# skitzoid/Box2D-MT

Measured on AMD Instinct MI355X. Metric: world steps/sec at 99858 bodies per GPU (BASELINE config 3: Tumbler 100k, CCD off; Step = collide + island solve + broad-phase + state read-back); for N > 1: container-steps/s = world steps/s x N containers in the one sharded world, higher is better.
Workload: dtype f32

## Files before the change

### box2d-mt_amd/csrc/b2d_kernels_broadphase.h

```cpp
#ifndef B2D_KERNELS_BROADPHASE_H
#define B2D_KERNELS_BROADPHASE_H

#include "b2d_kernels_solve_large.h"

#define SYNC_TILE 1024
__global__ __launch_bounds__(256) void k_sync_fixtures(DW W)
{
	b2dPhaseStamp(W);
	DState* S = W.st;
	const int n = W.nProxies;
	const int tid = (int)threadIdx.x;
	__shared__ int s_list[SYNC_TILE];
	__shared__ int s_cnt, s_base;
	const int perLane = n >= 262144 ? SYNC_TILE / 256 : 1, tile = 256 * perLane;
	if (blockIdx.x == 0 && tid == 0) S->c.gridFresh = 0;
	for (int base = blockIdx.x * tile; base < n; base += gridDim.x * tile)
	{
		if (tid == 0) s_cnt = 0;
		__syncthreads();
		for (int j = 0; j < perLane; ++j)
		{
			const int p = base + j * 256 + tid;
			if (p >= n) break;
			const int body = W.p_body[p];
// ... 124 lines not shown
			int ix, iy;
			proxyCell(W, a, &ix, &iy);
			atomicAdd(&W.gridCount[cellHash(ix, iy, W.gridMask)], 1);
		}
	}
}

__global__ __launch_bounds__(256) void k_grid_fill(DW W, int force)
{
	b2dPhaseStamp(W);
	DState* S = W.st;
	if (S->c.nMoves == 0 && !force) return;
	if (force == 1 && S->c.gridFresh) return;
	const int n = W.nProxies;
	for (int p = blockIdx.x * blockDim.x + threadIdx.x; p < n; p += gridDim.x * blockDim.x)
	{
		if (W.p_body[p] < 0) continue;
		float4 a = W.p_fat[p];
		if (proxyIsLarge(W, a)) continue;
		int ix, iy;
		proxyCell(W, a, &ix, &iy);
		uint32_t h = cellHash(ix, iy, W.gridMask);
		const int slot = W.gridStart[h] + atomicAdd(&W.gridCursor[h], 1);
		W.gridItems[slot] = p;
		W.gridFat[slot] = a;
	}
}

__device__ __forceinline__ bool pairPasses(const DW& W, int p, int q, uint64_t* keyOut, int2* proxOut)
{
	const int bodyP = W.p_body[p], bodyQ = W.p_body[q];
	if (bodyP == bodyQ) return false;
	if (W.spatial)
	{
		const bool mineP = (W.b_flags[bodyP] & BF_TYPE_MASK) != BT_STATIC && W.b_owner[bodyP] == (uint8_t)W.shardRank;
		const bool mineQ = (W.b_flags[bodyQ] & BF_TYPE_MASK) != BT_STATIC && W.b_owner[bodyQ] == (uint8_t)W.shardRank;
		if (!mineP && !mineQ) return false;
	}
	const int keyP = W.p_key[p], keyQ = W.p_key[q];
	const int lo = keyP < keyQ ? p : q;
	const int hi = keyP < keyQ ? q : p;
	const uint64_t key = ((uint64_t)(uint32_t)W.p_key[lo] << 32) | (uint32_t)W.p_key[hi];
	if (htContains(W, key + 1ull)) return false;
	if (!bodiesShouldCollide(W, W.p_body[hi], W.p_body[lo])) return false;
	if (!W.userFilter && !filterShouldCollide(W.p_filter0[lo], W.p_filter1[lo], W.p_filter0[hi], W.p_filter1[hi])) return false;
	if (b2dContactSwap(W.shapes[W.p_shape[lo]].type, W.shapes[W.p_shape[hi]].type) < 0) return false;
	*keyOut = key;
	*proxOut = make_int2(lo, hi);
	return true;
}

__device__ __forceinline__ void tryEmitPair(const DW& W, DState* S, int p, int q)
{
	uint64_t key;
	int2 prox;
	if (!pairPasses(W, p, q, &key, &prox)) return;
	int k = atomicAdd(&S->c.nPairs, 1);
	if (k < W.capPairs)
	{
		W.pairKey[k] = key;
		W.pairProxy[k] = prox;
	}
	else
	{
		atomicOr(&S->c.overflow, 2);
	}
}

#define PAIR_STAGE_CAP 256
struct PairStage
{
	uint64_t* key;
	int2* prox;
	int n;
// ... 39 lines not shown
	__syncthreads();
	pairStageStore(W, S, st, lane, s_stageBase + s_stageCount[wv]);
	st.n = 0;
}

struct PairHits
{
	int2* list;
	int n;
};
__device__ __forceinline__ void pairHitsFlush(const DW& W, DState* S, PairHits& h, PairStage& st, int lane)
{
	if (h.n == 0) return;
	if (st.n + h.n > PAIR_STAGE_CAP) pairStageDrain(W, S, st, lane);
	__builtin_amdgcn_fence(__ATOMIC_RELEASE, "wavefront");
	__builtin_amdgcn_wave_barrier();
	__builtin_amdgcn_fence(__ATOMIC_ACQUIRE, "wavefront");
	uint64_t key = 0ull;
	int2 prox = make_int2(0, 0);
	bool ok = false;
	if (lane < h.n)
	{
		const int2 pq = h.list[lane];
		ok = pairPasses(W, pq.x, pq.y, &key, &prox);
	}
	const unsigned long long om = __ballot(ok);
	if (ok)
	{
		const int j = st.n + (int)__popcll(om & ((1ull << lane) - 1ull));
		st.key[j] = key;
		st.prox[j] = prox;
	}
	st.n += (int)__popcll(om);
	__builtin_amdgcn_wave_barrier();
	h.n = 0;
}
__device__ __forceinline__ void pairHitsAdd(const DW& W, DState* S, PairHits& h, PairStage& st, int lane, bool hit, int p, int q)
{
	const unsigned long long hm = __ballot(hit);
	if (hm == 0ull) return;
	const int more = (int)__popcll(hm);
	if (h.n + more > 64) pairHitsFlush(W, S, h, st, lane);
	if (hit) h.list[h.n + (int)__popcll(hm & ((1ull << lane) - 1ull))] = make_int2(p, q);
	h.n += more;
}

__global__ __launch_bounds__(256) void k_find_pairs_small(DW W)
{
	b2dPhaseStamp(W);
	DState* S = W.st;
	const int nm = S->c.nMoves < W.capMoves ? S->c.nMoves : W.capMoves;
	const int nLarge = S->c.nLargeProxies;
	const int lane = (int)(threadIdx.x & 63u);
	const int waveId = (int)((blockIdx.x * blockDim.x + threadIdx.x) >> 6);
	const int nWaves = (int)((gridDim.x * blockDim.x) >> 6);
	int rounds = 0;
	__shared__ int2 s_hits[4][64];
	__shared__ uint64_t s_stageKey[4][PAIR_STAGE_CAP];
	__shared__ int2 s_stageProx[4][PAIR_STAGE_CAP];
	PairHits hits;
	hits.list = s_hits[threadIdx.x >> 6];
	hits.n = 0;
	PairStage stage;
	stage.key = s_stageKey[threadIdx.x >> 6];
	stage.prox = s_stageProx[threadIdx.x >> 6];
	stage.n = 0;
	const int largeQ = lane < nLarge ? W.largeProxies[lane] : -1;
	const float4 largeFat = largeQ >= 0 ? W.p_fat[largeQ] : make_float4(0, 0, 0, 0);
	auto cellHeaders = [&](const float4& f, int* cntOut, int* startOut)
	{
// ... 49 lines not shown
		for (int c = 0; c < 9; ++c)
		{
			ccs[c] = __builtin_amdgcn_readlane(cnt, c);
			scs[c] = __builtin_amdgcn_readlane(start, c);
			ecs[c] = total;
			total += ccs[c];
		}
		{ const int r = (total + 63) >> 6; rounds += r < 8 ? r : 8; }
		for (int base = 0; base < total; base += 64)
		{
			const int idx = base + lane;
			const bool valid = idx < total;
			int t = -1;
#pragma unroll
			for (int c = 0; c < 9; ++c)
			{
				const int ec = ecs[c], cc = ccs[c], sc = scs[c];
				if (valid && idx >= ec && idx < ec + cc) t = sc + (idx - ec);
			}
			bool hit = false;
			int q = -1;
			if (t >= 0)
			{
				q = W.gridItems[t];
				const float4 fq = W.gridFat[t];
				AABB bq;
				bq.lo = v2(fq.x, fq.y);
				bq.hi = v2(fq.z, fq.w);
				hit = q != p && b2dAabbOverlap(a, bq);
			}
			pairHitsAdd(W, S, hits, stage, lane, hit, p, q);
		}
		{
			AABB bq;
			bq.lo = v2(largeFat.x, largeFat.y);
			bq.hi = v2(largeFat.z, largeFat.w);
			pairHitsAdd(W, S, hits, stage, lane, largeQ >= 0 && b2dAabbOverlap(a, bq), p, largeQ);
		}
		for (int t = 64 + lane; t < nLarge; t += 64)
		{
			const int q = W.largeProxies[t];
			if (b2dAabbOverlap(a, loadAabb(W.p_fat, q))) tryEmitPair(W, S, p, q);
		}
	}
	pairHitsFlush(W, S, hits, stage, lane);
	pairStageFinish(W, S, stage, lane);
	b2dBlockTreeAdd2(W, ARRIVE_PAIRS, &S->c.candRounds[0], lane == 0 ? rounds : 0, &S->c.candRounds[1], 0, (unsigned)W.capMoves <= (TREE_SUM_MAX >> 3));
}


__global__ __launch_bounds__(256) void k_find_pairs_window(DW W)
{
	b2dPhaseStamp(W);
	DState* S = W.st;
	const int nm = S->c.nMoves < W.capMoves ? S->c.nMoves : W.capMoves;
	const int nLarge = S->c.nLargeProxies;
	const int lane = (int)(threadIdx.x & 63u);
	const int waveId = (int)((blockIdx.x * blockDim.x + threadIdx.x) >> 6);
	const int nWaves = (int)((gridDim.x * blockDim.x) >> 6);
	int rounds = 0;
	__shared__ int2 s_hits[4][64];
	__shared__ uint64_t s_stageKey[4][PAIR_STAGE_CAP];
	__shared__ int2 s_stageProx[4][PAIR_STAGE_CAP];
	PairHits hits;
	hits.list = s_hits[threadIdx.x >> 6];
	hits.n = 0;
	PairStage stage;
	stage.key = s_stageKey[threadIdx.x >> 6];
	stage.prox = s_stageProx[threadIdx.x >> 6];
	stage.n = 0;
	const int largeQ = lane < nLarge ? W.largeProxies[lane] : -1;
	const float4 largeFat = largeQ >= 0 ? W.p_fat[largeQ] : make_float4(0, 0, 0, 0);
	int pNext = waveId < nm ? W.moveBuf[waveId] : -1;
	int pAhead = waveId + nWaves < nm ? W.moveBuf[waveId + nWaves] : -1;
// ... 41 lines not shown
		{ const int r = (total + 63) >> 6; rounds += r < 8 ? r : 8; }
		for (int base = 0; base < total; base += 64)
		{
			const int idx = base + lane;
			const bool valid = idx < total;
			int t = -1;
			{
				int lo = 0, hi = nCells - 1;
#pragma unroll
				for (int step = 0; step < 6; ++step)
				{
					const int mid = (lo + hi) >> 1;
					const int im = __shfl(incl, mid);
					if (im > idx) hi = mid; else lo = mid + 1;
				}
				const int c = lo < 63 ? lo : 63;
				const int ec = __shfl(excl, c), sc = __shfl(start, c);
				if (valid) t = sc + (idx - ec);
			}
			bool hit = false;
			int q = -1;
			if (t >= 0)
			{
				q = W.gridItems[t];
				const float4 fq = W.gridFat[t];
				AABB bq;
				bq.lo = v2(fq.x, fq.y);
				bq.hi = v2(fq.z, fq.w);
				hit = q != p && b2dAabbOverlap(a, bq);
			}
			pairHitsAdd(W, S, hits, stage, lane, hit, p, q);
		}
		{
			AABB bq;
			bq.lo = v2(largeFat.x, largeFat.y);
			bq.hi = v2(largeFat.z, largeFat.w);
			pairHitsAdd(W, S, hits, stage, lane, largeQ >= 0 && b2dAabbOverlap(a, bq), p, largeQ);
		}
		for (int t = 64 + lane; t < nLarge; t += 64)
		{
			const int q = W.largeProxies[t];
			if (b2dAabbOverlap(a, loadAabb(W.p_fat, q))) tryEmitPair(W, S, p, q);
		}
	}
	pairHitsFlush(W, S, hits, stage, lane);
	pairStageFinish(W, S, stage, lane);
	b2dBlockTreeAdd2(W, ARRIVE_PAIRS, &S->c.candRounds[0], lane == 0 ? rounds : 0, &S->c.candRounds[1], 0, (unsigned)W.capMoves <= (TREE_SUM_MAX >> 3));
}

__global__ __launch_bounds__(256) void k_find_pairs_large(DW W)
{
	b2dPhaseStamp(W);
// ... 456 lines not shown
```

### box2d-mt_amd/csrc/b2d_kernels_query.h

```cpp
#ifndef B2D_KERNELS_QUERY_H
#define B2D_KERNELS_QUERY_H

#include "b2d_kernels_broadphase.h"
#include "b2d_kernels_collide.h"
#include "b2d_shapecast.h"
#include "b2d_shape_geom.h"

#define QUERY_WINDOW_MAX 4096
#define QUERY_COORD_MAX 1.0e8f
#define QUERY_SORT_MAX 4096
#define QUERY_SORT_THREADS 256

__device__ __forceinline__ bool queryFilterPasses(const DW& W, int q, uint32_t mask, int sensors)
{
	return (W.p_filter0[q] & mask & 0xffffu) != 0u && (sensors || (W.p_filter1[q] & PF_SENSOR) == 0);
}

__device__ __forceinline__ bool queryBoxSane(float4 b)
{
	return fabsf(b.x) <= QUERY_COORD_MAX && fabsf(b.y) <= QUERY_COORD_MAX && fabsf(b.z) <= QUERY_COORD_MAX && fabsf(b.w) <= QUERY_COORD_MAX;
}

__device__ __forceinline__ unsigned long long queryKey(uint32_t valueBits, int q)
{
// ... 57 lines not shown
			const int v = __shfl_up(incl, off);
			if (lane >= off) incl += v;
		}
		const int excl = incl - cnt;
		const int total = __shfl(incl, 63);
		for (int base = 0; base < total; base += 64)
		{
			const int idx = base + lane;
			int lo = 0, hi = 63;
#pragma unroll
			for (int step = 0; step < 6; ++step)
			{
				const int mid = (lo + hi) >> 1;
				if (__shfl(incl, mid) > idx) hi = mid; else lo = mid + 1;
			}
			const int cl = lo < 63 ? lo : 63;
			const int t = __shfl(start, cl) + (idx - __shfl(excl, cl));
			const int cellX = __shfl(cx, cl), cellY = __shfl(cy, cl);
			bool valid = idx < total;
			int q = -1;
			float4 fat = make_float4(0.0f, 0.0f, 0.0f, 0.0f);
			if (valid)
			{
				q = W.gridItems[t];
				fat = W.gridFat[t];
				int px, py;
				proxyCell(W, fat, &px, &py);
				valid = px == cellX && py == cellY;
			}
			visit(valid, q, fat);
		}
	}
	return true;
}

template <typename F>
__device__ __forceinline__ void queryVisitLarge(const DW& W, int lane, F& visit)
{
	const int nLarge = W.st->c.nLargeProxies;
	for (int base = 0; base < nLarge; base += 64)
	{
		const int k = base + lane;
		const int q = k < nLarge ? W.largeProxies[k] : -1;
		visit(q >= 0, q, q >= 0 ? W.p_fat[q] : make_float4(0.0f, 0.0f, 0.0f, 0.0f));
	}
}

// ... 666 lines not shown
```

### box2d-mt_amd/csrc/b2d_kernels_toi.h

```cpp
#ifndef B2D_KERNELS_TOI_H
#define B2D_KERNELS_TOI_H

#include "b2d_kernels_broadphase.h"
#include "b2d_toi.h"

#define TOI_LANES 512
#define TOI_CAND_MAX 512
#define TOI_MOVES_MAX 128
#define TOI_PAIRS_MAX 512
#define TOI_RECOMP_MAX 512
#define TOI_WOKEN_MAX 256
#define TOI_EVENTS_MAX 100000
#define TOI_NEWPAIR_MAX 256
#define TOI_MOVED_ALL_MAX 32768

__device__ __forceinline__ uint32_t ldFlags(const uint32_t* p)
{
	return __hip_atomic_load(p, __ATOMIC_RELAXED, __HIP_MEMORY_SCOPE_AGENT);
}

__device__ __forceinline__ Sweep loadSweep(const DW& W, int body)
{
	const float4 p0 = W.b_pos0[body], p = W.b_pos[body], m = W.b_mass[body];
	Sweep s;
	s.localCenter = v2(m.z, m.w);
	s.c0 = v2(p0.x, p0.y);
	s.a0 = p0.z;
	s.alpha0 = p0.w;
	s.c = v2(p.x, p.y);
	s.a = p.z;
	return s;
}

template <typename F>
__device__ __forceinline__ void toiForEachCandidate(const DW& W, AABB a, int lane, int nLanes, const int* moved, int nMoved, F f)
{
	int ix0, iy0, nx, ny;
	if (!gridWindow(W, make_float4(a.lo.x, a.lo.y, a.hi.x, a.hi.y), &ix0, &iy0, &nx, &ny))
	{
		for (int q = lane; q < W.nProxies; q += nLanes) f(q);
		return;
	}
	const int nCells = nx * ny;
	for (int c = lane; c < nCells; c += nLanes)
	{
		const uint32_t h = cellHash(ix0 + c % nx, iy0 + c / nx, W.gridMask);
		const int start = W.gridStart[h], n = W.gridCount[h];
		for (int t = 0; t < n; ++t) f(W.gridItems[start + t]);
	}
	const int nLarge = W.st->c.nLargeProxies;
	for (int t = lane; t < nLarge; t += nLanes) f(W.largeProxies[t]);
	for (int t = lane; t < nMoved; t += nLanes) f(moved[t]);
}

__device__ __forceinline__ float computeToiOf(const GjkProxy& pA, const GjkProxy& pB, const Sweep& sA, const Sweep& sB)
{
	float t = 1.0f;
	const int state = b2dTimeOfImpact(&t, pA, sA, pB, sB, 1.0f);
	const float alpha0 = sA.alpha0;
	return state == TOI_TOUCHING ? b2dMin(alpha0 + (1.0f - alpha0) * t, 1.0f) : 1.0f;
}
__device__ __forceinline__ float computeToi(const DW& W, int4 ids, const Sweep& sA, const Sweep& sB)
{
	const GjkProxy pA = b2dProxy(W.shapes + W.p_shape[ids.x]);
	const GjkProxy pB = b2dProxy(W.shapes + W.p_shape[ids.y]);
	float t = 1.0f;
	const int state = b2dTimeOfImpact(&t, pA, sA, pB, sB, 1.0f);
	const float alpha0 = sA.alpha0;
	return state == TOI_TOUCHING ? b2dMin(alpha0 + (1.0f - alpha0) * t, 1.0f) : 1.0f;
}

// ... 1211 lines not shown
```

### box2d-mt_amd/csrc/b2d_kernels_toi_chains.h

```cpp
#ifndef B2D_KERNELS_TOI_CHAINS_H
#define B2D_KERNELS_TOI_CHAINS_H

#include "b2d_kernels_toi.h"

#define CHAIN_LANES 64
#define CHAIN_CAND_MAX 64
#define CHAIN_EVENTS_MAX 4096
#define CHAIN_ADJ_MAX 32
#define TOI_GROUPS_MAX 262144

#define TOI_UNSAFE_PARTNER 1
#define TOI_UNSAFE_WOKE 2
#define TOI_UNSAFE_PAIR 4
#define TOI_UNSAFE_CAPACITY 8
#define TOI_UNSAFE_MOVED 16

__global__ __launch_bounds__(256) void k_toi_groups_begin(DW W)
{
	b2dPhaseStamp(W);
	DState* S = W.st;
	const int n = S->c.nToiList < W.capContacts ? S->c.nToiList : W.capContacts;
	const ContactArrays& C = W.ca[S->cur];
	for (int k = blockIdx.x * blockDim.x + threadIdx.x; k < n; k += gridDim.x * blockDim.x)
	{
// ... 778 lines not shown
			if (events) atomicAdd(&S->c.nToiEvents, (int)events);
			if (calls) atomicAdd(&S->c.nToiCalls, (int)calls);
		}
		toiChainsEnd(W);
	}
}

__global__ __launch_bounds__(256) void k_bp_clear(DW W)
{
	b2dPhaseStamp(W);
	DState* S = W.st;
	if (blockIdx.x == 0 && threadIdx.x == 0)
	{
		S->c.nLargeProxies = 0;
		S->c.nLargeMoves = 0;
		S->c.nPairs = 0;
		S->c.nNewContacts = 0;
		S->c.nMovesSeen = S->c.nMoves;
		S->c.gridFresh = S->c.nMoves != 0 ? 1 : 0;
	}
	if (blockIdx.x == 0 && threadIdx.x < 32) S->c.candRounds[threadIdx.x] = 0;
	if (S->c.nMoves == 0) return;
	const uint32_t stride = gridDim.x * blockDim.x, t0 = blockIdx.x * blockDim.x + threadIdx.x;
	{
		const float cap = 4.0f * W.cellSize;
		float ext = 0.0f;
		for (uint32_t p = t0; p < (uint32_t)W.nProxies; p += stride)
		{
			if (W.p_body[p] < 0) continue;
			const float4 a = W.p_fat[p];
			const float e = fmaxf(a.z - a.x, a.w - a.y);
			if (e <= cap && e > ext) ext = e;
		}
		blockAtomicMaxIfAbove((int*)&S->c.cellExtBits, ext > 0.0f ? (int)__float_as_uint(ext) : 0);
	}
	{
		const int4 z = make_int4(0, 0, 0, 0);
		int4* gc = (int4*)W.gridCount;
		int4* gu = (int4*)W.gridCursor;
		for (uint32_t i = t0, n4 = (W.gridMask + 1u) >> 2; i < n4; i += stride)
		{
			gc[i] = z;
			gu[i] = z;
		}
		if (keysetDecision(W) != 0)
		{
// ... 42 lines not shown
```

### box2d-mt_amd/csrc/b2d_world.h

```cpp
#ifndef B2D_WORLD_H
#define B2D_WORLD_H

#include "b2d_solver.h"
#include "b2d_joint.h"
#include "b2d_wave.h"

#define BF_TYPE_MASK 0x3u
#define BF_AWAKE 0x4u
#define BF_AUTOSLEEP 0x8u
#define BF_BULLET 0x10u
#define BF_FIXEDROT 0x20u
#define BF_ACTIVE 0x40u
#define BF_ISLAND 0x80u
#define BF_LARGE 0x100u

#define BT_STATIC 0u
#define BT_KINEMATIC 1u
#define BT_DYNAMIC 2u

#define CF_TOUCHING 0x1u
#define CF_ENABLED 0x2u
#define CF_FILTER 0x4u
#define CF_TOI_CANDIDATE 0x8u
#define CF_SENSOR 0x10u
// ... 369 lines not shown
	int4* spTailKey;
	int userFilter;
	int preSolveOn, postSolveOn;
	float4* pre_o0;
	float4* pre_o1;
	float4* pre_oimp;
	int4* pre_o3;
	PreSolveRec* preRecs;
	PostSolveRec* postRecs;
	ToiLogRec* toiLog;
	int capToiLog;
	int toiEventCap;
	int toiContinue;
	const int4* toiVerdict;
	int nToiVerdict;
	int* filterList;

	int* moveBuf;
	int* gridCount;
	int* gridStart;
	int* gridCursor;
	unsigned long long* arriveTree;
	int* gridItems;
	float4* gridFat;
	int* largeProxies;
	int* largeMoves;
	uint64_t* pairKey;
	int2* pairProxy;
	uint64_t* pairKey2;
	int2* pairProxy2;
	int* pairFirst;
	int* pairRank;

	int* toiList;
	int* toiPos2c;
	int* toiDestroyList;
	int* toiNewList;
	int* b_toiGroup;
	int* toiGroups;
	int* toiParent;
	int* toiDomOf;
	int* toiDomRoot;
	int* toiDomCount;
	int* toiDomBase;
	int* toiDomFill;
	int* toiDomList;
	int* toiDomFailed;
	int* toiDomEvents;
	float4* toiHull;
	int* toiGroupCount;
	int* toiGroupList;
	int* toiMoved;
	int gridHalf;
	int noOwnIdBlocks;
	int noChainCreate;
	int* toiNew;
	float4* snapBody;
	float4* snapFat;

	int* scanTmp;
	int* radixHist;
	int* keepFlag;
	int* keepScan;

	float* stateOut;
};

#if defined(__HIPCC__)
__host__ __device__ inline bool b2dPartitionSettled(const Counters& c)
{
	if (c.nBlocks == 0 || c.nOrphanRows > 0 || c.blkMaxRows > c.blkLanes || c.blkMaxBodies > c.blkLanes || c.nSerialOrphans > 2048) return false;
	if (c.partitionAge > 240 && (4 * c.nCutRows > c.nLContacts || 2 * c.nLContacts < 900)) return false;
	return true;
}

__device__ __forceinline__ void b2dStoreAgentI(int* p, int v) { __hip_atomic_store(p, v, __ATOMIC_RELAXED, __HIP_MEMORY_SCOPE_AGENT); }
__device__ __forceinline__ int b2dLoadAgentI(const int* p) { return __hip_atomic_load(p, __ATOMIC_RELAXED, __HIP_MEMORY_SCOPE_AGENT); }
__device__ __forceinline__ void b2dStoreAgent4(float4* p, float4 v)
{
	typedef float f4 __attribute__((ext_vector_type(4)));
	f4 q;
	q.x = v.x; q.y = v.y; q.z = v.z; q.w = v.w;
	asm volatile("global_store_dwordx4 %0, %1, off sc1\n\ts_nop 1" :: "v"(p), "v"(q) : "memory");
}
__device__ __forceinline__ float4 b2dLoadAgent4(const float4* p)
{
	typedef float f4 __attribute__((ext_vector_type(4)));
	f4 r;
	asm volatile("global_load_dwordx4 %0, %1, off sc1\n\ts_waitcnt vmcnt(0)" : "=v"(r) : "v"(p) : "memory");
	return make_float4(r.x, r.y, r.z, r.w);
}
// ... 119 lines not shown
```

### box2d-mt_amd/csrc/b2hip_api_callbacks.h

```cpp

int b2hip_set_contact_filter(b2hip_world* w, b2hip_should_collide_fn fn, void* user)
{
	if (int rcu = checkUsable(w, "b2hip_set_contact_filter", true)) return rcu;
	w->filterFn = fn;
	w->filterUser = user;
	w->dw.userFilter = hasFilter(w) ? 1 : 0;
	return B2HIP_OK;
}

int b2hip_set_contact_filter_batch(b2hip_world* w, b2hip_should_collide_batch_fn fn, void* user)
{
	if (int rcu = checkUsable(w, "b2hip_set_contact_filter_batch", true)) return rcu;
	w->filterBatchFn = fn;
	if (fn) w->filterUser = user;
	w->dw.userFilter = hasFilter(w) ? 1 : 0;
	return B2HIP_OK;
}

int b2hip_default_should_collide(b2hip_world* w, int fixture_a, int fixture_b)
{
	if (!w || fixture_a < 0 || fixture_b < 0 || fixture_a >= (int)w->fixtures.size() || fixture_b >= (int)w->fixtures.size())
		return setError(B2HIP_ERR_INVALID, "bad fixture id");
	const HostFixture& a = w->fixtures[fixture_a];
	const HostFixture& b = w->fixtures[fixture_b];
// ... 212 lines not shown
	case 31:
	{
		if (first != 0 || count != 1) return setError(B2HIP_ERR_INVALID, "island-build statistics: [0, 1)");
		memcpy(out, &w->statUnionSkipped, sizeof(long long));
		return 0;
	}
	case 29:
	{
		if (first != 0 || count != 1) return setError(B2HIP_ERR_INVALID, "lifecycle statistics: [0, 1)");
		memcpy(out, &w->statLifecycleLongSorts, sizeof(long long));
		return 0;
	}
	case 30:
	{
		const long long stats[2] = { w->statFixtureLongSorts, w->statFixtureRelists };
		if (first < 0 || count < 0 || first + count > 2) return setError(B2HIP_ERR_INVALID, "fixture-batch statistics: [0, 2)");
		memcpy(out, stats + first, (size_t)count * sizeof(long long));
		return 0;
	}
	case 32:
	{
		if (first != 0 || count != 1) return setError(B2HIP_ERR_INVALID, "body-property statistics: [0, 1)");
		memcpy(out, &w->statBodyPropRefits, sizeof(long long));
		return 0;
	}
	case 25:
	{
		if (first < 0 || count < 0 || first + count > ToiStats::N) return setError(B2HIP_ERR_INVALID, "TOI host statistics: [0, 10)");
		memcpy(out, w->toiStats.n + first, (size_t)count * sizeof(long long));
		return 0;
	}
	case 26:
	{
		const int nb = (int)std::min(w->bodies.size(), w->upBodies);
		if (first < 0 || count < 0 || first + count > nb) return setError(B2HIP_ERR_INVALID, "effective blocks: [0, uploaded bodies)");
		if (count == 0) return 0;
		if (!w->d_state.p || !w->b_blk1.p || !w->b_adopt.p || !w->b_flags.p) return setError(B2HIP_ERR_INVALID, "effective blocks: nothing uploaded yet");
		Counters c;
		HIP_TRY(hipMemcpy(&c, &w->d_state.p->c, sizeof(Counters), hipMemcpyDeviceToHost));
		std::vector<int> blk1((size_t)count), adopt((size_t)count);
		std::vector<uint32_t> flags((size_t)count);
		HIP_TRY(hipMemcpy(blk1.data(), w->b_blk1.p + first, (size_t)count * sizeof(int), hipMemcpyDeviceToHost));
		HIP_TRY(hipMemcpy(adopt.data(), w->b_adopt.p + first, (size_t)count * sizeof(int), hipMemcpyDeviceToHost));
		HIP_TRY(hipMemcpy(flags.data(), w->b_flags.p + first, (size_t)count * sizeof(uint32_t), hipMemcpyDeviceToHost));
		const int blocks = c.nBlocks < MAX_BLOCKS ? c.nBlocks : MAX_BLOCKS;
		const bool ownIdOff = (w->dw.nJoints != 0 || c.maxDegree > HUB_DEGREE) && w->dw.noOwnIdBlocks >= 0;
// ... 309 lines not shown
```

### box2d-mt_amd/csrc/b2hip_api_snapshot.h

```cpp

namespace
{
struct SnapHeader
{
	char magic[8];
	uint32_t version, szDState, szHostBody, szHostFixture, szShape, szJoint;
	uint32_t nBodies, nFixtures, nShapes, nJoints, nFree, nContacts, nToiOrder, nMoves;
	uint32_t stateCount, cur;
	int32_t nextNode, leafCount, lastContacts, newFixture;
	float inv_dt0, cellSize;
	int32_t eventsOn, solverHints;
};
const uint32_t kSnapVersion = 6;
const char kSnapMagic[8] = { 'B', '2', 'H', 'I', 'P', 'S', 'N', '1' };

struct SnapWriter
{
	std::vector<char> out;
	void host(const void* p, size_t n) { const char* c = (const char*)p; out.insert(out.end(), c, c + n); }
	int dev(const void* p, size_t n)
	{
		const size_t at = out.size();
		out.resize(at + n);
		if (n == 0) return 0;
// ... 260 lines not shown
	w->gears.resize(nG);
	if (nG) memcpy((void*)w->gears.data(), gearsAt, nG * sizeof(GearRec));
	w->nextNode = h.nextNode; w->leafCount = h.leafCount; w->lastContacts = h.lastContacts; w->newFixture = h.newFixture != 0;
	w->inv_dt0 = h.inv_dt0;
	w->eventsOn = h.eventsOn != 0;
	w->serialOrphansNext = h.solverHints & 1;
	w->blocksTooBig = (h.solverHints & 2) != 0;
	w->stepComplete = (h.solverHints & 4) == 0;
	w->adoptSticky = (h.solverHints >> 8) & 0xff;
	w->largeHintSteps = (h.solverHints >> 16) & 0xff;
	w->recolorCountdown = (h.solverHints >> 24) & 0x7f;
	w->freshColors = ((h.solverHints >> 3) & 0x1f) | ((int)(((uint32_t)h.solverHints >> 31) & 1u) << 5);
	w->freshColorsPending = false;
	w->adoptPasses = w->adoptSticky > 0;
	rc = ensureCapacity(w, nC);
	if (rc) return fail(rc);
	if (nM > w->moveBuf.cap || nC > (size_t)w->dw.capContacts || (size_t)h.stateCount * 10 > w->h_stateCap) return fail(corrupt("counts exceed the buffers sized for them"));
	if (h.stateCount) memcpy(w->h_state, stateAt, (size_t)h.stateCount * 10 * sizeof(float));
	w->shadowDev = nullptr;
	w->stateCount = h.stateCount;
	*w->h_dstate = ds;
	w->contactsKnown = false;
	forestDrop(w);
#define SNAP_UP(arr, s) do { if ((s).bytes && hipMemcpy(w->arr.p, (s).p, (s).bytes, hipMemcpyHostToDevice) != hipSuccess) return fail(setError(B2HIP_ERR_HIP, "snapshot upload failed (" #arr ")")); } while (0)
	if (hipMemcpy(w->d_state.p, &ds, sizeof(DState), hipMemcpyHostToDevice) != hipSuccess) return fail(setError(B2HIP_ERR_HIP, "snapshot upload failed (state block)"));
	w->pubSeq = ds.pubCount;
	SNAP_UP(b_pos, sPos); SNAP_UP(b_pos0, sPos0); SNAP_UP(b_vel, sVel); SNAP_UP(b_xf, sXf); SNAP_UP(b_mass, sMass); SNAP_UP(b_damp, sDamp);
	w->forceOnDevice = true; w->rowsWentEarly = false;
	SNAP_UP(b_force, sForce); SNAP_UP(b_flags, sFlags); SNAP_UP(b_wake, sWake); SNAP_UP(b_proxyHead, sHead); SNAP_UP(b_blk1, sBlk);
	SNAP_UP(p_fat, sFat); SNAP_UP(p_body, sPBody); SNAP_UP(p_shape, sPShape); SNAP_UP(p_key, sPKey); SNAP_UP(p_filter0, sF0); SNAP_UP(p_filter1, sF1);
	SNAP_UP(p_mat, sPMat); SNAP_UP(p_next, sNext);
	const int cur = (int)h.cur;
	SNAP_UP(c_ids[cur], cIds); SNAP_UP(c_key[cur], cKey); SNAP_UP(c_flags[cur], cFlags); SNAP_UP(c_mat[cur], cMat); SNAP_UP(c_man0[cur], cMan0);
	SNAP_UP(c_man1[cur], cMan1); SNAP_UP(c_imp[cur], cImp); SNAP_UP(c_man3[cur], cMan3); SNAP_UP(c_color[cur], cColor); SNAP_UP(c_mgr[cur], cMgr);
	SNAP_UP(toiPos2c, sToi); SNAP_UP(moveBuf, sMoves);
#undef SNAP_UP
	if (nS && hipMemcpy(w->d_shapes.p, w->shapes.data(), nS * sizeof(ShapeRec), hipMemcpyHostToDevice) != hipSuccess)
		return fail(setError(B2HIP_ERR_HIP, "snapshot upload failed (shapes)"));
	w->upBodies = nb; w->upFixtures = np; w->upShapes = nS; w->upJoints = 0;
	w->dw.cellSize = h.cellSize;
	w->dw.invCellSize = 1.0f / h.cellSize;
	w->dw.eventsOn = w->eventsOn ? 1 : 0;
	*out = w;
	return B2HIP_OK;
}

// ... 48 lines not shown
```

### box2d-mt_amd/csrc/b2hip_host_phases.h

```cpp

static int spExchangeState(b2hip_world* w, int mode);
static int spExchangePairs(b2hip_world* w, long long* totalPairs, int* straddling);
static int spResolve(b2hip_world* w, int nVirt = 0);
static int spAfterToi(b2hip_world* w);
static int spBeginStep(b2hip_world* w);

static int radixBits(int maxKey)
{
	int bits = 1;
	while ((1 << bits) <= maxKey && bits < 31) ++bits;
	return bits;
}

static void radixPasses(int first, int bits, std::vector<std::pair<int, int>>& out)
{
	const int passes = (bits + RADIX_BITS - 1) / RADIX_BITS;
	for (int p = 0, at = 0; p < passes; ++p)
	{
		const int width = (bits - at + (passes - p) - 1) / (passes - p);
		out.push_back(std::make_pair(first + at, width));
		at += width;
	}
}

// ... 140 lines not shown
	if (c.overflow & 2) w->pairCapHint = 2 * (size_t)c.nPairs + 4096;
	int rc = ensureCapacity(w, (size_t)c.nContacts + (size_t)std::max(c.nNewContacts, 0) + 1024);
	if (rc) return rc;
	HIP_TRY(hipMemsetAsync(&w->d_state.p->c.overflow, 0, sizeof(int), w->stream));
	return 0;
}

static int findNewContacts(b2hip_world* w, bool sync)
{
	w->contactsKnown = false;
	forestDrop(w);
	for (int attempt = 0; sync && attempt < 4; ++attempt)
	{
		int rc = findNewContactsOnce(w, true);
		if (rc != 1) return rc;
	}
	if (sync) return setError(B2HIP_ERR_CAPACITY, "pair buffer overflow");
	return findNewContactsOnce(w, false);
}

static int findNewContactsOnce(b2hip_world* w, bool sync)
{
	DW& d = w->dw;
	LAUNCH(w, k_bp_clear, gridFor(std::max(d.htMask, d.gridMask) + 1), 256, d);
	LAUNCH(w, k_bp_build, gridFor(std::max(d.capContacts, d.nProxies)), 256, d);
	deviceExclusiveScan<int>(w->stream, d.gridCount, d.gridStart, d.scanTmp, w->scanCtx, w->consts.p + 1, (int)(d.gridMask + 1));
	LAUNCH(w, k_grid_fill, gridFor(d.nProxies), 256, d, 0);
	if (int rk = ktBracket(w, 4, 7)) return rk;
	if (d.gridHalf) LAUNCH(w, k_find_pairs_window, gridFor((size_t)d.capMoves * 64, 256, 2048), 256, d);
	else LAUNCH(w, k_find_pairs_small, gridFor((size_t)d.capMoves * 64, 256, 2048), 256, d);
	if (int rk = ktBracket(w, 4, 7)) return rk;
	LAUNCH(w, k_find_pairs_large, 1024, 256, d);
	bool large = false;
	if (w->spatial)
	{
		long long total = 0;
		int straddle = 0;
		int rc = spExchangePairs(w, &total, &straddle);
		if (rc) return rc;
		large = total > COUNT_RANK_MAX;
		rc = runSortAndCreate(w, large, total);
		if (rc) return rc;
		if (straddle == 0)
		{
			HIP_TRY(hipMemsetAsync(&w->d_state.p->c.nStraddle, 0, 4 * sizeof(int), w->stream));
			LAUNCH(w, k_sp_flag_contacts, gridFor(d.capContacts), 256, d);
// ... 1108 lines not shown
```

### box2d-mt_amd/csrc/b2hip_host_world.h

```cpp

static thread_local std::string g_lastError;

static int setError(int code, const std::string& msg)
{
	g_lastError = msg;
	return code;
}

#define HIP_TRY(expr)                                                                                   \
	do                                                                                                  \
	{                                                                                                   \
		hipError_t _e = (expr);                                                                         \
		if (_e != hipSuccess)                                                                           \
		{                                                                                               \
			return setError(B2HIP_ERR_HIP, std::string(#expr) + ": " + hipGetErrorString(_e));          \
		}                                                                                               \
	} while (0)

static void (*g_rcclDestroy)(void* comm) = nullptr;

static std::atomic<long long> g_liveBlocks{0};

template <typename T>
struct DevArray
// ... 237 lines not shown
	X(float4, b_posv, z.nb, true, true) \
	X(unsigned long long, evKey, z.cc, true, true) \
	X(int4, evInfo, z.cc, true, true) \
	X(int, uncolList, COLOR_SMALL_MAX, true, true) \
	X(int, compactList, COLOR_SMALL_MAX, true, true) \
	X(int, hubRowOf, z.cc, true, true) \
	X(int, hubList, z.cc, true, true) \
	X(float4, hubDelta, z.cc, true, true) \
	X(unsigned long long, hubMeta, 8, true, true) \
	X(unsigned long long, hubFirst, z.nb, true, true) \
	X(float4, solveSnapBody, w->recoverOn ? 6 * z.nb : 1, true, true) \
	X(float4, solveSnapImp, w->recoverOn ? z.cc : 1, true, true) \
	X(uint32_t, solveSnapCFlags, w->recoverOn ? z.cc : 1, true, true) \
	X(uint32_t, rootPen, ROOT_PEN_SLOTS * z.nb, true, true) \
	X(int, rootDone, z.nb, true, true) \
	X(uint32_t, rootSleepMin, z.nb, true, true) \
	X(float, lc, (size_t)LC_WORDS * z.cc, false, false) \
	X(float4, warmDelta, 4 * z.cc, false, false)  \
	X(int, moveBuf, 2 * z.np + 64, true, true) \
	X(int, gridCount, z.gridSize, true, true) \
	X(int, gridStart, z.gridSize + 2, true, true) \
	X(int, gridCursor, z.gridSize, true, true) \
	X(int, gridItems, z.np, true, true) \
	X(float4, gridFat, z.np, true, true) \
	X(unsigned long long, arriveTree, (size_t)ARRIVE_SITES * TREE_WORDS, true, true) \
	X(int, largeProxies, z.np, true, true) \
	X(int, largeMoves, 2 * z.np + 64, true, true) \
	X(uint64_t, pairKey, z.capPairs, true, true) \
	X(uint64_t, pairKey2, z.capPairs, true, true) \
	X(int2, pairProxy, z.capPairs, true, true) \
	X(int2, pairProxy2, z.capPairs, true, true) \
	X(int, pairFirst, z.capPairs + 1, true, true) \
	X(int, pairRank, z.capPairs + 2, true, true) \
	X(int, radixHist, RADIX_DIGITS * z.radixTiles + 2, true, true) \
	X(int, scanTmp, 3 * (std::max(z.maxScanN, RADIX_DIGITS * z.radixTiles) / SCAN_TILE + 8), true, true) \
	X(int, keepFlag, z.cc + 1, true, true) \
	X(int, keepScan, z.cc + 2, true, true) \
	X(int, toiList, z.cc, true, true) \
	X(int, toiPos2c, z.cc, true, true) \
	X(int, toiDestroyList, z.cc, true, true) \
	X(int, toiNewList, TOI_NEW_LIST_MAX, true, true) \
	X(int, b_toiGroup, z.nb, true, true) \
	X(int, toiGroups, z.nb, true, true) \
	X(int, toiGroupCount, std::min<size_t>(z.nb, TOI_GROUPS_MAX), true, true) \
	X(int, toiGroupList, std::min<size_t>(z.nb, TOI_GROUPS_MAX) * CHAIN_ADJ_MAX, true, true) \
	X(int, toiMoved, TOI_MOVED_ALL_MAX, true, true) \
// ... 185 lines not shown
	int spToiUnsafe = 0;
	bool spToiSettled = false;
	bool spTapeRecord = false;
	std::vector<std::pair<int*, size_t> > spTape;
	b2hip_world* spTapeFrom = nullptr;
	size_t spTapeCursor = 0;
	long long spToiRedos = 0;
	size_t spUp = 0;
	ScanFlags scanCtx = {};
	RadixStatus radixCtx = {};
	bool sortOnepass = true;
	long long statSorts = 0, statSortsOnepass = 0;
	int dfEpoch = 0;
	bool noSideStream = false, profileDetail = false;
	int collideStage = -1;
	int solidRoundsEnv = 0;
	int collideSplitEnv = -1;
	bool collideCompactOn = true;
	int collideChunk = 256;
	bool contactsKnown = false;
	unsigned collideEpoch = 0;
	long long statCollideCompact = 0;
	bool collideUnionOn = true;
	bool forestUnited = false;
	bool forestVoided = false;
	long long statUnionSkipped = 0;
	bool collideUniOff = false;
	int collideSortEnv = -1;
	hipStream_t stream2 = nullptr;
	hipEvent_t evFork = nullptr, evJoin = nullptr;
	DevArray<unsigned long long> filterPairs;
	std::vector<int> nonStatic;
	bool orderDirty = false;
	std::vector<int2> editOps;
	std::vector<int> proxyEdits;
	std::vector<int> fatEdits;
	bool proxyListsStale = false;
	DevArray<int2> d_editOps;
	b2hip_should_collide_fn filterFn = nullptr;
	void* filterUser = nullptr;
	bool refilterPending = false;
	b2hip_pre_solve_fn preSolveFn = nullptr;
	b2hip_pre_solve_batch_fn preSolveBatchFn = nullptr;
	b2hip_should_collide_batch_fn filterBatchFn = nullptr;
	void* preSolveUser = nullptr;
	bool postSolveOn = false;
// ... 537 lines not shown
	if (int rc = pollPublished(w, (volatile const int*)&w->h_pub->pubSeq, w->pubSeq, "island census")) return rc;
	memcpy(w->h_dstate, w->h_pub, offsetof(DState, pubSeq));
	return 0;
}

static bool envSet(const char* k) { return getenv(k) != nullptr; }
static bool envOn(const char* k) { const char* e = getenv(k); return e && atoi(e); }
static int envInt(const char* k, int unset) { const char* e = getenv(k); return e ? atoi(e) : unset; }

static void readSwitches(b2hip_world* w)
{
	DW& d = w->dw;
	w->debugSync = envSet("B2HIP_DEBUG");
	w->traceLaunches = envSet("B2HIP_TRACE_LAUNCHES");
	w->debugTrace = envSet("B2HIP_TRACE");
	w->forceLarge = envInt("B2HIP_FORCE_LARGE", 0);
	w->kernelTimingLaunches = envSet("B2HIP_SOLVER_LAUNCHES");
	w->noSideStream = envSet("B2HIP_NO_SIDE_STREAM");
	w->profileDetail = envInt("B2HIP_PROFILE_DETAIL", 1) != 0;
	if (const char* e = getenv("B2HIP_SOLID_ROUNDS")) { const int v = atoi(e); w->solidRoundsEnv = (v == 1 || v == 2 || v == 4 || v == 8) ? v : 0; }
	w->collideSplitEnv = envInt("B2HIP_COLLIDE_SPLIT", -1);
	w->collideCompactOn = envInt("B2HIP_COLLIDE_COMPACT", 1) != 0;
	w->collideUnionOn = envInt("B2HIP_COLLIDE_UNION", 1) != 0;
	w->collideChunk = std::min(std::max(envInt("B2HIP_TEST_COLLIDE_CHUNK", 256), 1), 256);
	w->lifecycleSortMax = std::min(std::max(envInt("B2HIP_TEST_LIFECYCLE_SORT_MAX", LIFECYCLE_SORT_MAX), 0), LIFECYCLE_SORT_MAX);
	w->fixtureListRoom = std::max(envInt("B2HIP_TEST_FIXTURE_LIST_ROOM", -1), -1);
	w->collideUniOff = envInt("B2HIP_COLLIDE_UNI", 1) == 0;
	w->collideSortEnv = envInt("B2HIP_COLLIDE_SORT", -1);
	w->sortOnepass = envInt("B2HIP_SORT_ONEPASS", 1) != 0;
	d.keysetKeep = envInt("B2HIP_KEYSET_KEEP", 1) != 0 ? 1 : 0;
	d.keysetMaxFill = std::min(std::max(envInt("B2HIP_KEYSET_MAX_FILL", 37), 1), 90);
	w->collideStage = envInt("B2HIP_COLLIDE_STAGE", -1);
	w->noSweepBlocks = envSet("B2HIP_NO_SWEEP_BLOCKS");
	w->tracePartition = envSet("B2HIP_TRACE_PARTITION");
	w->traceRecovery = envSet("B2HIP_TRACE_RECOVERY");
	if (const char* e = getenv("B2HIP_GRID_HALF")) { w->gridForced = true; w->gridHalf = atoi(e) != 0; d.gridHalf = w->gridHalf ? 1 : 0; }
	d.noChainCreate = envSet("B2HIP_TOI_NO_CHAIN_CREATE") ? 1 : 0;
	d.noOwnIdBlocks = envSet("B2HIP_NO_OWN_ID_BLOCKS") ? 1 : envSet("B2HIP_OWN_ID_BLOCKS_ALL") ? -1 : 0;
	w->noBlocks = envSet("B2HIP_NO_BLOCKS");
	w->blockLanes = 0;
	if (const char* e = getenv("B2HIP_BLOCK_LANES")) w->blockLanes = atoi(e) == 512 ? 512 : (atoi(e) == 256 ? 256 : (atoi(e) == 1024 ? 1024 : 0));
	w->toiSw.serialOnly = envSet("B2HIP_TOI_SERIAL");
	w->toiSw.syncOnly = envSet("B2HIP_TOI_SYNC");
	w->toiSw.domWideOnly = envSet("B2HIP_TOI_DOM_WIDE");
	w->toiSw.noSpecDomains = envSet("B2HIP_TOI_NO_SPEC_DOMAINS");
	w->toiSw.assumeFreshGrid = envSet("B2HIP_DEBUG_ASSUME_FRESH_GRID");
// ... 147 lines not shown
```

Before: 385.0.

## Emit each moved-moved pair once and batch pair filter loads in broad-phase

Stamps each moved proxy with a per-step epoch and tags its grid item with a high bit, so when two moved proxies overlap, only the lower-index side emits the pair. This removes duplicate candidate pairs that were previously filtered later by hash lookups. A new pairPassesRounds loads all filter inputs up front and evaluates them branch-light, and the pair-finding kernels get an occupancy hint in launch_bounds. It adds a stamp array, an extra write pass over moved proxies, and epoch bookkeeping, and it is disabled during graph capture and spatial sharding.

```diff
diff --git a/box2d-mt_amd/csrc/b2d_kernels_broadphase.h b/box2d-mt_amd/csrc/b2d_kernels_broadphase.h
--- a/box2d-mt_amd/csrc/b2d_kernels_broadphase.h
+++ b/box2d-mt_amd/csrc/b2d_kernels_broadphase.h
@@ -170,7 +170,8 @@
 		proxyCell(W, a, &ix, &iy);
 		uint32_t h = cellHash(ix, iy, W.gridMask);
 		const int slot = W.gridStart[h] + atomicAdd(&W.gridCursor[h], 1);
-		W.gridItems[slot] = p;
+		const bool moved = force == 0 && W.pairEpoch != 0u && W.movedStamp[p] == W.pairEpoch;
+		W.gridItems[slot] = moved ? (int)((uint32_t)p | GRID_ITEM_MOVED) : p;
 		W.gridFat[slot] = a;
 	}
 }
@@ -198,6 +199,60 @@
 	return true;
 }
 
+__device__ __forceinline__ bool pairPassesRounds(const DW& W, int p, int q, uint64_t* keyOut, int2* proxOut)
+{
+	const int bodyP = W.p_body[p], bodyQ = W.p_body[q];
+	const int keyP = W.p_key[p], keyQ = W.p_key[q];
+	const uint32_t f0P = W.p_filter0[p], f0Q = W.p_filter0[q];
+	const int f1P = W.p_filter1[p], f1Q = W.p_filter1[q];
+	const int shapeP = W.p_shape[p], shapeQ = W.p_shape[q];
+	const bool pLow = keyP < keyQ;
+	const int lo = pLow ? p : q, hi = pLow ? q : p;
+	const uint64_t key = ((uint64_t)(uint32_t)(pLow ? keyP : keyQ) << 32) | (uint32_t)(pLow ? keyQ : keyP);
+	const int bodyLo = pLow ? bodyP : bodyQ, bodyHi = pLow ? bodyQ : bodyP;
+	const uint32_t ksMask = W.st->c.ksMask;
+	uint32_t h = hashKey(key + 1ull) & ksMask;
+	const uint64_t slot0 = W.ht_keys[h];
+	const uint32_t flagsLo = W.b_flags[bodyLo], flagsHi = W.b_flags[bodyHi];
+	int e = 0, end = 0;
+	if (W.nJoints != 0)
+	{
+		e = W.jadjStart[bodyHi];
+		end = W.jadjStart[bodyHi + 1];
+	}
+	const int typeLo = W.shapes[pLow ? shapeP : shapeQ].type, typeHi = W.shapes[pLow ? shapeQ : shapeP].type;
+	bool ok = bodyP != bodyQ;
+	const bool walk = ok & (slot0 != key + 1ull) & (slot0 != 0ull);
+	ok &= slot0 != key + 1ull;
+	ok &= (flagsHi & BF_TYPE_MASK) == BT_DYNAMIC || (flagsLo & BF_TYPE_MASK) == BT_DYNAMIC;
+	ok &= W.userFilter != 0 || filterShouldCollide(pLow ? f0P : f0Q, pLow ? f1P : f1Q, pLow ? f0Q : f0P, pLow ? f1Q : f1P);
+	ok &= b2dContactSwap(typeLo, typeHi) >= 0;
+	if (walk)
+	{
+		bool found = false, open = true;
+		for (uint32_t probes = 1; open && probes <= ksMask; ++probes)
+		{
+			h = (h + 1) & ksMask;
+			const uint64_t v = W.ht_keys[h];
+			found = v == key + 1ull;
+			open = !found && v != 0ull;
+		}
+		if (open) W.st->c.ksStale = 1;
+		ok &= !found;
+	}
+	if (ok)
+	{
+		for (; e < end; ++e)
+		{
+			const JointRec& jn = W.joints[W.jadj[e]];
+			if ((jn.bodyA == bodyLo || jn.bodyB == bodyLo) && jn.collideConnected == 0) ok = false;
+		}
+	}
+	*keyOut = key;
+	*proxOut = make_int2(lo, hi);
+	return ok;
+}
+
 __device__ __forceinline__ void tryEmitPair(const DW& W, DState* S, int p, int q)
 {
 	uint64_t key;
@@ -283,7 +338,7 @@
 	if (lane < h.n)
 	{
 		const int2 pq = h.list[lane];
-		ok = pairPasses(W, pq.x, pq.y, &key, &prox);
+		ok = W.pairEpoch != 0u ? pairPassesRounds(W, pq.x, pq.y, &key, &prox) : pairPasses(W, pq.x, pq.y, &key, &prox);
 	}
 	const unsigned long long om = __ballot(ok);
 	if (ok)
@@ -306,7 +361,7 @@
 	h.n += more;
 }
 
-__global__ __launch_bounds__(256) void k_find_pairs_small(DW W)
+__global__ __launch_bounds__(256, 6) void k_find_pairs_small(DW W)
 {
 	b2dPhaseStamp(W);
 	DState* S = W.st;
@@ -402,12 +457,13 @@
 			int q = -1;
 			if (t >= 0)
 			{
-				q = W.gridItems[t];
+				const int item = W.gridItems[t];
+				q = gridItemProxy(item);
 				const float4 fq = W.gridFat[t];
 				AABB bq;
 				bq.lo = v2(fq.x, fq.y);
 				bq.hi = v2(fq.z, fq.w);
-				hit = q != p && b2dAabbOverlap(a, bq);
+				hit = q != p && !(item < 0 && q < p) && b2dAabbOverlap(a, bq);
 			}
 			pairHitsAdd(W, S, hits, stage, lane, hit, p, q);
 		}
@@ -429,7 +485,7 @@
 }
 
 
-__global__ __launch_bounds__(256) void k_find_pairs_window(DW W)
+__global__ __launch_bounds__(256, 6) void k_find_pairs_window(DW W)
 {
 	b2dPhaseStamp(W);
 	DState* S = W.st;
@@ -517,12 +573,13 @@
 			int q = -1;
 			if (t >= 0)
 			{
-				q = W.gridItems[t];
+				const int item = W.gridItems[t];
+				q = gridItemProxy(item);
 				const float4 fq = W.gridFat[t];
 				AABB bq;
 				bq.lo = v2(fq.x, fq.y);
 				bq.hi = v2(fq.z, fq.w);
-				hit = q != p && b2dAabbOverlap(a, bq);
+				hit = q != p && !(item < 0 && q < p) && b2dAabbOverlap(a, bq);
 			}
 			pairHitsAdd(W, S, hits, stage, lane, hit, p, q);
 		}
diff --git a/box2d-mt_amd/csrc/b2d_kernels_query.h b/box2d-mt_amd/csrc/b2d_kernels_query.h
--- a/box2d-mt_amd/csrc/b2d_kernels_query.h
+++ b/box2d-mt_amd/csrc/b2d_kernels_query.h
@@ -103,7 +103,7 @@
 			float4 fat = make_float4(0.0f, 0.0f, 0.0f, 0.0f);
 			if (valid)
 			{
-				q = W.gridItems[t];
+				q = gridItemProxy(W.gridItems[t]);
 				fat = W.gridFat[t];
 				int px, py;
 				proxyCell(W, fat, &px, &py);
diff --git a/box2d-mt_amd/csrc/b2d_kernels_toi.h b/box2d-mt_amd/csrc/b2d_kernels_toi.h
--- a/box2d-mt_amd/csrc/b2d_kernels_toi.h
+++ b/box2d-mt_amd/csrc/b2d_kernels_toi.h
@@ -46,7 +46,7 @@
 	{
 		const uint32_t h = cellHash(ix0 + c % nx, iy0 + c / nx, W.gridMask);
 		const int start = W.gridStart[h], n = W.gridCount[h];
-		for (int t = 0; t < n; ++t) f(W.gridItems[start + t]);
+		for (int t = 0; t < n; ++t) f(gridItemProxy(W.gridItems[start + t]));
 	}
 	const int nLarge = W.st->c.nLargeProxies;
 	for (int t = lane; t < nLarge; t += nLanes) f(W.largeProxies[t]);
diff --git a/box2d-mt_amd/csrc/b2d_kernels_toi_chains.h b/box2d-mt_amd/csrc/b2d_kernels_toi_chains.h
--- a/box2d-mt_amd/csrc/b2d_kernels_toi_chains.h
+++ b/box2d-mt_amd/csrc/b2d_kernels_toi_chains.h
@@ -824,6 +824,15 @@
 	if (blockIdx.x == 0 && threadIdx.x < 32) S->c.candRounds[threadIdx.x] = 0;
 	if (S->c.nMoves == 0) return;
 	const uint32_t stride = gridDim.x * blockDim.x, t0 = blockIdx.x * blockDim.x + threadIdx.x;
+	if (W.pairEpoch != 0u)
+	{
+		const uint32_t nm = (uint32_t)(S->c.nMoves < W.capMoves ? S->c.nMoves : W.capMoves);
+		for (uint32_t k = t0; k < nm; k += stride)
+		{
+			const int p = W.moveBuf[k];
+			if ((unsigned)p < (unsigned)W.nProxies) W.movedStamp[p] = W.pairEpoch;
+		}
+	}
 	{
 		const float cap = 4.0f * W.cellSize;
 		float ext = 0.0f;
diff --git a/box2d-mt_amd/csrc/b2d_world.h b/box2d-mt_amd/csrc/b2d_world.h
--- a/box2d-mt_amd/csrc/b2d_world.h
+++ b/box2d-mt_amd/csrc/b2d_world.h
@@ -415,6 +415,8 @@
 	int* gridCursor;
 	unsigned long long* arriveTree;
 	int* gridItems;
+	uint32_t* movedStamp;
+	uint32_t pairEpoch;
 	float4* gridFat;
 	int* largeProxies;
 	int* largeMoves;
@@ -460,6 +462,9 @@
 };
 
 #if defined(__HIPCC__)
+#define GRID_ITEM_MOVED 0x80000000u
+__host__ __device__ inline int gridItemProxy(int item) { return (int)((uint32_t)item & ~GRID_ITEM_MOVED); }
+
 __host__ __device__ inline bool b2dPartitionSettled(const Counters& c)
 {
 	if (c.nBlocks == 0 || c.nOrphanRows > 0 || c.blkMaxRows > c.blkLanes || c.blkMaxBodies > c.blkLanes || c.nSerialOrphans > 2048) return false;
diff --git a/box2d-mt_amd/csrc/b2hip_api_callbacks.h b/box2d-mt_amd/csrc/b2hip_api_callbacks.h
--- a/box2d-mt_amd/csrc/b2hip_api_callbacks.h
+++ b/box2d-mt_amd/csrc/b2hip_api_callbacks.h
@@ -258,6 +258,16 @@
 	{
 		if (first != 0 || count != 1) return setError(B2HIP_ERR_INVALID, "body-property statistics: [0, 1)");
 		memcpy(out, &w->statBodyPropRefits, sizeof(long long));
+		return 0;
+	}
+	case 33:
+	{
+		if (first < 0 || count < 0 || first + count > 2) return setError(B2HIP_ERR_INVALID, "pair-search statistics: [0, 2)");
+		if (!w->d_state.p) return setError(B2HIP_ERR_INVALID, "pair-search statistics: nothing uploaded yet");
+		Counters c;
+		HIP_TRY(hipMemcpy(&c, &w->d_state.p->c, sizeof(Counters), hipMemcpyDeviceToHost));
+		const long long stats[2] = { c.nNewContacts, std::min(c.nPairs, w->dw.capPairs) };
+		memcpy(out, stats + first, (size_t)count * sizeof(long long));
 		return 0;
 	}
 	case 25:
diff --git a/box2d-mt_amd/csrc/b2hip_api_snapshot.h b/box2d-mt_amd/csrc/b2hip_api_snapshot.h
--- a/box2d-mt_amd/csrc/b2hip_api_snapshot.h
+++ b/box2d-mt_amd/csrc/b2hip_api_snapshot.h
@@ -306,6 +306,9 @@
 	*w->h_dstate = ds;
 	w->contactsKnown = false;
 	forestDrop(w);
+	if (w->movedStamp.p && hipMemsetAsync(w->movedStamp.p, 0, w->movedStamp.cap * sizeof(uint32_t), w->stream) != hipSuccess)
+		return fail(setError(B2HIP_ERR_HIP, "snapshot load failed (moved stamps)"));
+	w->pairEpoch = 0u;
 #define SNAP_UP(arr, s) do { if ((s).bytes && hipMemcpy(w->arr.p, (s).p, (s).bytes, hipMemcpyHostToDevice) != hipSuccess) return fail(setError(B2HIP_ERR_HIP, "snapshot upload failed (" #arr ")")); } while (0)
 	if (hipMemcpy(w->d_state.p, &ds, sizeof(DState), hipMemcpyHostToDevice) != hipSuccess) return fail(setError(B2HIP_ERR_HIP, "snapshot upload failed (state block)"));
 	w->pubSeq = ds.pubCount;
diff --git a/box2d-mt_amd/csrc/b2hip_host_phases.h b/box2d-mt_amd/csrc/b2hip_host_phases.h
--- a/box2d-mt_amd/csrc/b2hip_host_phases.h
+++ b/box2d-mt_amd/csrc/b2hip_host_phases.h
@@ -186,6 +186,21 @@
 static int findNewContactsOnce(b2hip_world* w, bool sync)
 {
 	DW& d = w->dw;
+	d.pairEpoch = 0u;
+	if (w->pairOnce != 0 && !w->spatial && w->movedStamp.p != nullptr)
+	{
+		hipStreamCaptureStatus capturing = hipStreamCaptureStatusNone;
+		(void)hipStreamIsCapturing(w->stream, &capturing);
+		if (capturing == hipStreamCaptureStatusNone)
+		{
+			if (w->pairEpoch >= 0xfffffffeu)
+			{
+				HIP_TRY(hipMemsetAsync(w->movedStamp.p, 0, w->movedStamp.cap * sizeof(uint32_t), w->stream));
+				w->pairEpoch = 0u;
+			}
+			d.pairEpoch = ++w->pairEpoch;
+		}
+	}
 	LAUNCH(w, k_bp_clear, gridFor(std::max(d.htMask, d.gridMask) + 1), 256, d);
 	LAUNCH(w, k_bp_build, gridFor(std::max(d.capContacts, d.nProxies)), 256, d);
 	deviceExclusiveScan<int>(w->stream, d.gridCount, d.gridStart, d.scanTmp, w->scanCtx, w->consts.p + 1, (int)(d.gridMask + 1));
diff --git a/box2d-mt_amd/csrc/b2hip_host_world.h b/box2d-mt_amd/csrc/b2hip_host_world.h
--- a/box2d-mt_amd/csrc/b2hip_host_world.h
+++ b/box2d-mt_amd/csrc/b2hip_host_world.h
@@ -283,6 +283,7 @@
 	X(int, gridStart, z.gridSize + 2, true, true) \
 	X(int, gridCursor, z.gridSize, true, true) \
 	X(int, gridItems, z.np, true, true) \
+	X(uint32_t, movedStamp, z.np, true, true) \
 	X(float4, gridFat, z.np, true, true) \
 	X(unsigned long long, arriveTree, (size_t)ARRIVE_SITES * TREE_WORDS, true, true) \
 	X(int, largeProxies, z.np, true, true) \
@@ -514,6 +515,8 @@
 	unsigned collideEpoch = 0;
 	long long statCollideCompact = 0;
 	bool collideUnionOn = true;
+	int pairOnce = 1;
+	uint32_t pairEpoch = 0;
 	bool forestUnited = false;
 	bool forestVoided = false;
 	long long statUnionSkipped = 0;
@@ -1097,6 +1100,8 @@
 	w->collideSplitEnv = envInt("B2HIP_COLLIDE_SPLIT", -1);
 	w->collideCompactOn = envInt("B2HIP_COLLIDE_COMPACT", 1) != 0;
 	w->collideUnionOn = envInt("B2HIP_COLLIDE_UNION", 1) != 0;
+	w->pairOnce = envInt("B2HIP_PAIR_ONCE", 1);
+	if (const char* e = getenv("B2HIP_TEST_PAIR_EPOCH")) w->pairEpoch = (uint32_t)strtoul(e, nullptr, 0);
 	w->collideChunk = std::min(std::max(envInt("B2HIP_TEST_COLLIDE_CHUNK", 256), 1), 256);
 	w->lifecycleSortMax = std::min(std::max(envInt("B2HIP_TEST_LIFECYCLE_SORT_MAX", LIFECYCLE_SORT_MAX), 0), LIFECYCLE_SORT_MAX);
 	w->fixtureListRoom = std::max(envInt("B2HIP_TEST_FIXTURE_LIST_ROOM", -1), -1);
```

New measurement: 364.1. 0.946x the previous value.
